# burmajam/delta_crdt_ex

Hardware: AMD Instinct MI355X
Metric: merged dots/sec for AWLWWMap delta join + Merkle diff keys/sec at 1–8 GPUs (higher is better)
Workload: dtype u64; 1 GPU; config2: 1M-key AWLWWMap full-state join of two replicas, 10% concurrent-write conflicts, per GPU (key-hash range shards); keys_per_gpu=1000000, rows_in_per_gpu=2000000, rows_out_per_gpu=1100011, parallelism=key-hash shards x1, rotate=4

## Files before the change

### delta_crdt_ex_amd/csrc/join.hip

```cpp
#include <algorithm>
#include <mutex>

#include "dg_ctxu.h"
#include "dg_launch.h"

namespace dg {

namespace {

constexpr int JB = JOIN_BLOCK;
constexpr int JI = JOIN_ITEMS;
constexpr int JT = JOIN_TILE;
static_assert(JT % 2 == 0, "even tiles (balance_tiles keeps them even)");
constexpr int JS = JT + 5;
constexpr int VT = 64;

#ifdef DG_STAMPS
__device__ u64 g_join_stamps[65536 * 16];
#define JSTAMP(tile, k)                                                              \
  do {                                                                               \
    __syncthreads();                                                                 \
    __builtin_amdgcn_sched_barrier(0);                                               \
    if (threadIdx.x == 0 && (tile) < 65536) g_join_stamps[(tile) * 16 + (k)] =       \
        __builtin_amdgcn_s_memrealtime();                                            \
    __builtin_amdgcn_sched_barrier(0);                                               \
  } while (0)
#else
#define JSTAMP(tile, k) \
  do {                  \
  } while (0)
#endif

constexpr int CB = 1024;

__global__ __launch_bounds__(CB) void ctx_union_kernel(CtxUnionArgs p) {
  __shared__ u32 s_wave[CB / WAVE + 1];
  ctx_union_block<CB>(p, s_wave);
}

struct ChgLayout {
  u64* ev;
  u64* off;
  u32* cnt;
  u32* wu;
  u64* fk;
  u64* lk;
};

static __host__ ChgLayout chg_layout(void* tmp, u64 ntiles) {
  ChgLayout l;
  char* c = (char*)tmp;
  l.ev = (u64*)c;
  c += ntiles * (u64)JT * 8;
  l.off = (u64*)c;
  c += ntiles * 8;
  l.cnt = (u32*)c;
  c += ntiles * 4;
  l.wu = (u32*)c;
  c += ntiles * 4;
  c += ntiles * 4;
  c = (char*)(((uintptr_t)c + 7) & ~(uintptr_t)7);
  l.fk = (u64*)c;
  c += ntiles * 8;
  l.lk = (u64*)c;
  return l;
}

struct JoinArgs {
  Rows a, b;
  Ctx ca, cb;
  const u64* keys;
  u64 n_keys;
  const u64* splits;
  u64* ksplits;
  u64 ntiles;
  u64 jt;
  RowsOut out;
  Scan scan;
  u64* d_count;
  unsigned short* lists;
  u32* counts;
  u64* chg_tmp;
  u32* chg_cnt;
  u32* chg_wu;
  u64* chg_fk;
  u64* chg_lk;
  int fused;
  CtxUnionArgs cu;
};

__device__ __forceinline__ bool mp_pred(const Rows A, const Rows B, u64 diag, u64 i) {
  u64 j = diag - 1 - i;
  u64 ka = A.key[i], kb = B.key[j];
  if (ka != kb) return ka < kb;
  return row_le(load_row(A, i), load_row(B, j));
}

constexpr int PB = 256;
constexpr int PK = 2 * WAVE;

__device__ u64 mp_search(const Rows A, const Rows B, u64 d, u64 lo, u64 hi) {
  const int lane = threadIdx.x & (WAVE - 1);
  for (int round = 0; round < 64 && hi > lo; round++) {
    const u64 span = hi - lo;
    bool f0, f1;
    if (span <= (u64)PK) {
      const u64 x0 = lo + 2 * lane, x1 = x0 + 1;
      f0 = x0 < hi && !mp_pred(A, B, d, x0);
      f1 = x1 < hi && !mp_pred(A, B, d, x1);
    } else {
      const u64 x0 = lo + (span * (u64)(2 * lane + 1)) / (PK + 1);
      const u64 x1 = lo + (span * (u64)(2 * lane + 2)) / (PK + 1);
      f0 = !mp_pred(A, B, d, x0);
      f1 = !mp_pred(A, B, d, x1);
    }
    const u64 m0 = __ballot(f0), m1 = __ballot(f1);
    int kf = PK;
    if (m0 | m1) {
      const int l0 = m0 ? __ffsll((long long)m0) - 1 : 64;
      const int l1 = m1 ? __ffsll((long long)m1) - 1 : 64;
      kf = (l0 <= l1) ? 2 * l0 : 2 * l1 + 1;
    }
    if (span <= (u64)PK) {
      return (u64)kf < span ? lo + kf : hi;
    } else if (kf == PK) {
      lo = lo + (span * (u64)PK) / (PK + 1) + 1;
    } else {
      const u64 nh = lo + (span * (u64)(kf + 1)) / (PK + 1);
      if (kf > 0) lo = lo + (span * (u64)kf) / (PK + 1) + 1;
      hi = nh;
    }
  }
  return lo;
}

__device__ u64 mp_split(const Rows A, const Rows B, u64 d) {
  const int lane = threadIdx.x & (WAVE - 1);
  const u64 na = A.n, nb = B.n, total = na + nb;
  const u64 lo = d > nb ? d - nb : 0, hi = min(d, na);
  if (hi - lo <= (u64)PK) return mp_search(A, B, d, lo, hi);
  const double scale = (double)na * (double)nb / ((double)total * 18446744073709551616.0);
  u64 i = (u64)((double)d * (double)na / (double)total);
  i = min(max(i, lo), hi - 1);
  {
    const double gap = (double)B.key[d - 1 - i] - (double)A.key[i];
    const double lim = (double)(hi - lo);
    double sft = gap * scale;
    sft = sft > lim ? lim : (sft < -lim ? -lim : sft);
    i64 ni = (i64)i + (i64)sft;
    ni = ni < (i64)lo ? (i64)lo : (ni > (i64)hi - 1 ? (i64)hi - 1 : ni);
    i = (u64)ni;
  }
  for (int r = 0; r < 3; r++) {
    constexpr u64 PW = WAVE;
    u64 wlo = i > lo + PW / 2 ? i - PW / 2 : lo;
    const u64 whi = min(wlo + PW, hi);
    wlo = whi - PW > lo ? whi - PW : lo;
    const u64 x0 = wlo + lane;
    const u64 m0 = __ballot(x0 < whi && !mp_pred(A, B, d, x0));
    const u64 kf = m0 ? (u64)(__ffsll((long long)m0) - 1) : whi - wlo;
    if ((kf > 0 || wlo == lo) && (kf < whi - wlo || whi == hi)) return wlo + kf;
    const u64 c = (wlo + whi) / 2;
    const double gap = (double)B.key[d - 1 - c] - (double)A.key[c];
    double sft = gap * scale;
    const double lim = (double)(hi - lo);
    sft = sft > lim ? lim : (sft < -lim ? -lim : sft);
    i64 ni = (i64)c + (i64)sft;
    ni = ni < (i64)lo ? (i64)lo : (ni > (i64)hi - 1 ? (i64)hi - 1 : ni);
    i = (u64)ni;
  }
  return mp_search(A, B, d, lo, hi);
}

__device__ __forceinline__ u64 split_guess(u64 na, u64 nb, u64 d) {
  const u64 lo = d > nb ? d - nb : 0, hi = min(d, na);
  const u64 i = (u64)((double)d * (double)na / (double)(na + nb));
  return min(max(i, lo), hi);
}

__device__ __forceinline__ bool guess_exact(const Rows& A, const Rows& B, u64 d, u64 g) {
  const u64 lo = d > B.n ? d - B.n : 0, hi = min(d, A.n);
  bool ok = true;
  if (g > lo) ok = row_le(load_row(A, g - 1), load_row(B, d - g));
  if (g < hi) ok = ok && !row_le(load_row(A, g), load_row(B, d - 1 - g));
  return ok;
}

__device__ __forceinline__ u64 key_split(const Rows& A, const Rows& B, const u64* keys, u64 n_keys,
                                         u64 d, u64 s) {
  const u64 ib = d - s;
  const bool va = s < A.n, vb = ib < B.n;
  if (!va && !vb) return n_keys;
  const u64 ka = va ? A.key[s] : ~0ull, kb = vb ? B.key[ib] : ~0ull;
  return wave_lower_bound(keys, n_keys, min(ka, kb));
}

__global__ __launch_bounds__(PB) void join2_partition_kernel(Rows A, Rows B, u64 ntiles, u64 jt,
                                                             u64* splits, CtxUnionArgs cu,
                                                             const u64* keys, u64 n_keys,
                                                             u64* ksplits) {
  if (blockIdx.x == 0) {
    __shared__ u32 s_wave[PB / WAVE + 1];
    ctx_union_block<PB>(cu, s_wave);
    return;
  }
  const u64 q = (u64)(blockIdx.x - 1) * (PB / WAVE) + (threadIdx.x >> 6);
  if (q > ntiles) return;
  const u64 d = min(q * jt, A.n + B.n);
  const u64 s = mp_split(A, B, d);
  if ((threadIdx.x & (WAVE - 1)) == 0) splits[q] = s;
  if (keys) {
    const u64 kq = key_split(A, B, keys, n_keys, d, s);
    if ((threadIdx.x & (WAVE - 1)) == 0) ksplits[q] = kq;
  }
}

template <bool FAST>
__device__ __forceinline__ bool covers(const u64* tab, const Ctx& c, u32 dn, u64 dc) {
  if (FAST) {
    if (dn < (u32)VT) return tab[dn] >= dc;
    return ctx_covers(c.node, c.cnt, c.n, 0, dn, dc);
  }
  return ctx_covers(c.node, c.cnt, c.n, c.kind, dn, dc);
}

constexpr int KS = 64;
struct KeySlice {
  const u64* lds;
  const u64* keys;
  u64 km;
};

__device__ __forceinline__ bool key_in(const KeySlice& ks, u64 x) {
  if (ks.lds) {
    const int km = (int)ks.km;
    int pos = 0;
#pragma unroll
    for (int step = KS; step >= 1; step >>= 1) {
      const int m = pos + step;
      const bool c = (m <= km) & (ks.lds[min(m, KS) - 1] < x);
      pos = c ? m : pos;
    }
    return (pos < km) & (ks.lds[min(pos, KS - 1)] == x);
  }
  return keyset_has(ks.keys, ks.km, x);
}

__device__ __forceinline__ bool fill_vv_tables(const Ctx& ca, const Ctx& cb, u64* tab_a, u64* tab_b) {
  bool far = false;
  for (u64 i = threadIdx.x; i < ca.n; i += JB) {
    const u32 nd = ca.node[i];
    if (nd < (u32)VT) tab_a[nd] = ca.cnt[i];
    far |= nd >= (u32)VT;
  }
  for (u64 i = threadIdx.x; i < cb.n; i += JB) {
    const u32 nd = cb.node[i];
    if (nd < (u32)VT) tab_b[nd] = cb.cnt[i];
    far |= nd >= (u32)VT;
  }
  return far;
}

struct Buf {
  alignas(16) u64 kv[JS][2];
  alignas(16) u64 tc[JS][2];
  u32 node[JS];
};

__device__ __forceinline__ u64 buf_key(const Buf& s, int x) { return s.kv[x][0]; }

__device__ __forceinline__ void buf_put(Buf& s, int x, u64 key, u64 val, i64 ts, u32 node, u64 cnt) {
  typedef u64 v2u64 __attribute__((ext_vector_type(2)));
  *(v2u64*)s.kv[x] = v2u64{key, val};
  *(v2u64*)s.tc[x] = v2u64{(u64)ts, cnt};
  s.node[x] = node;
}

__device__ __forceinline__ i64 slot_row(int x, int nat, u64 a0, u64 b0, u64 na, u64 nb,
                                        bool* from_b) {
  if (x < nat + 2) {
    const i64 g = (i64)a0 - 1 + x;
    *from_b = false;
    return (g >= 0 && (u64)g < na) ? g : -1;
  }
  const i64 g = (i64)b0 - 1 + (x - (nat + 2));
  *from_b = true;
  return (g >= 0 && (u64)g < nb) ? g : -1;
}

constexpr int SLOTS = (JS + JB - 1) / JB;

__device__ __forceinline__ Row lds_row(const Buf& s, int x) {
  typedef u64 v2u64 __attribute__((ext_vector_type(2)));
  const v2u64 kv = *(const v2u64*)s.kv[x];
  const v2u64 tc = *(const v2u64*)s.tc[x];
  Row r;
  r.key = kv.x;
  r.val = kv.y;
  r.ts = (i64)tc.x;
  r.cnt = tc.y;
  r.node = s.node[x];
  return r;
}

constexpr int search_top(int n) { return n <= 1 ? 1 : 2 * search_top(n / 2); }
constexpr int STOP = search_top(JT);

template <bool FAST, bool KEYED, bool CHG = false, bool NOFB = false>
__device__ __forceinline__ void merge_items(const Ctx& ca, const Ctx& cb, const u64* tab_a,
                                            const u64* tab_b, const KeySlice& ks,
                                            const u64 nb, const Buf& s, int nat, int nbt, u64 a0,
                                            u64 b0, u32& keep, unsigned short (&src)[JI],
                                            u32* ev = nullptr) {
  const int tid = threadIdx.x;
  const int offB = nat + 2;
  const int tt = nat + nbt;
  const int diag = min(tid * JI, tt);
  const int dend = min(diag + JI, tt);
  const int lo0 = diag > nbt ? diag - nbt : 0, hi0 = min(diag, nat);
  int lo = lo0;
#pragma unroll
  for (int step = STOP; step >= 1; step >>= 1) {
    const int m = lo + step;
    const int mc = min(m, hi0);
    const bool c = (m <= hi0) & (buf_key(s, mc) <= buf_key(s, offB + 1 + diag - mc));
    lo = c ? m : lo;
  }
  int i = lo;
  while (i > lo0 && buf_key(s, i) == buf_key(s, offB + 1 + diag - i)) {
    bool lt, eq;
    row_cmp_bf(lds_row(s, i), lds_row(s, offB + 1 + diag - i), lt, eq);
    if (lt | eq) break;
    i--;
  }
  int j = diag - i;
  Row ra = lds_row(s, 1 + i), rb = lds_row(s, offB + 1 + j);
  bool dup = false;
  if (((a0 + (u64)i) >= 1) && buf_key(s, i) == rb.key) dup = row_eq(lds_row(s, i), rb);
  Row xa = lds_row(s, 2 + i), xb = lds_row(s, offB + 2 + j);
  keep = 0;
  if (CHG) *ev = 0;
#pragma unroll
  for (int k = 0; k < JI; k++) {
    const bool valid = diag + k < dend;
    const bool bvalid = (b0 + (u64)j) < nb;
    bool lt, eq;
    row_cmp_bf(ra, rb, lt, eq);
    const bool takeA = (i < nat) & ((j >= nbt) | lt | eq);
    const bool inB = bvalid & eq;
    bool kp;
    const bool jn = KEYED ? key_in(ks, takeA ? ra.key : rb.key) : true;
    if (FAST) {
      const u32 dn = takeA ? ra.node : rb.node;
      const u64 dc = takeA ? ra.cnt : rb.cnt;
      bool cov;
      if (dn < (u32)VT) {
        cov = (takeA ? tab_b : tab_a)[dn] >= dc;
      } else if (NOFB) {
        cov = dc == 0;
      } else {
        const u32* vn = takeA ? opaque_ptr(cb.node) : opaque_ptr(ca.node);
        const u64* vc = takeA ? opaque_ptr(cb.cnt) : opaque_ptr(ca.cnt);
        const u64 vnn = takeA ? opaque_val(cb.n) : opaque_val(ca.n);
        cov = ctx_covers(vn, vc, vnn, 0, dn, dc);
      }
      if (KEYED) {
        const bool bprev = ((b0 + (u64)j) >= 1) & (buf_key(s, offB + j) == ra.key);
        const bool bnext = bvalid & (rb.key == ra.key);
        kp = takeA ? (jn ? (inB | !cov) : !(bprev | bnext)) : (!jn | (!dup & !cov));
      } else {
        kp = takeA ? (inB || !cov) : (!dup && !cov);
      }
    } else if (takeA) {
      if (jn) {
        kp = inB || !covers<FAST>(tab_b, cb, ra.node, ra.cnt);
      } else {
        const bool bprev = (b0 + (u64)j) >= 1 && buf_key(s, offB + j) == ra.key;
        const bool bnext = bvalid && rb.key == ra.key;
        kp = !(bprev || bnext);
      }
    } else {
      if (jn)
        kp = !dup && !covers<FAST>(tab_a, ca, rb.node, rb.cnt);
      else
        kp = true;
    }
    src[k] = valid ? (unsigned short)(takeA ? 1 + i : offB + 1 + j) : (unsigned short)0;
    if (valid && kp) keep |= 1u << k;
    if (CHG && valid && jn && (takeA ? !kp : kp)) *ev |= 1u << k;
    dup = takeA ? inB : false;
    i += takeA ? 1 : 0;
    j += takeA ? 0 : 1;
    ra = row_sel(takeA, xa, ra);
    rb = row_sel(takeA, rb, xb);
    if (k + 1 < JI) {
      const Row nx = lds_row(s, takeA ? 2 + i : offB + 2 + j);
      xa = row_sel(takeA, nx, xa);
      xb = row_sel(takeA, xb, nx);
    }
  }
}

struct TileLds {
  Buf buf;
  union {
    u64 tab[2][VT];
    unsigned short comp[JT];
  } u;
  u32 wave[JB / WAVE + 1];
  u64 lb[3 * (JB / WAVE) + 2];
  u64 bcast[4];
};

struct Staged {
  u64 k[SLOTS], v[SLOTS], c[SLOTS];
  i64 t[SLOTS];
  u32 n[SLOTS];
  bool ok[SLOTS];
};

__device__ __forceinline__ void tile_geom(u64 t, u64 jt, u64 a0, u64 a1, u64 total, int* nat,
                                          int* nbt, u64* b0) {
  const u64 d0 = t * jt, d1 = min(d0 + jt, total);
  *nat = (int)(a1 - a0);
  *nbt = (int)((d1 - a1) - (d0 - a0));
  *b0 = d0 - a0;
}

__device__ __forceinline__ void issue_tile(const Rows& A, const Rows& B, int nat, int nbt, u64 a0,
                                           u64 b0, Staged& r) {
  const int tid = threadIdx.x;
#pragma unroll
  for (int k = 0; k < SLOTS; k++) {
    const int x = tid + k * JB;
    bool fb = false;
    const i64 g = x < nat + nbt + 4 ? slot_row(x, nat, a0, b0, A.n, B.n, &fb) : -1;
    r.ok[k] = g >= 0;
    if (r.ok[k]) {
      const Row x = load_row_sel(A, B, fb, (u64)g);
      r.k[k] = x.key;
      r.v[k] = x.val;
      r.t[k] = x.ts;
      r.n[k] = x.node;
      r.c[k] = x.cnt;
    }
  }
}

__device__ __forceinline__ void commit_tile(const Staged& r, Buf& s) {
  const int tid = threadIdx.x;
#pragma unroll
  for (int k = 0; k < SLOTS; k++) {
    const int x = tid + k * JB;
    if (r.ok[k]) buf_put(s, x, r.k[k], r.v[k], r.t[k], r.n[k], r.c[k]);
  }
}

constexpr int FUSE_IT = 4;

template <bool KEYED>
struct StreamLds {
  Buf buf[2];
  unsigned short comp[2][JT];
  u64 tab[2][VT];
  u64 kslice[2][KEYED ? KS : 1];
  u64 kspl[KEYED ? 2 * FUSE_IT : 1];
  u32 wave[JB / WAVE + 1];
  u64 red[2][2 * (JB / WAVE)];
  u64 spl[2 * FUSE_IT];
  u64 chk[JB / WAVE];
  int chf[JB / WAVE];
};

constexpr u32 CNT_BITS = 12;
static_assert(JT < (1 << CNT_BITS), "tile count must fit the granule's count field");
constexpr int CQ = (1024 + JB - 1) / JB;
static_assert((u64)CQ * JB + 1 <= JOIN_MAX_GRID, "start flags cover every join grid");

__device__ __forceinline__ void publish_count(u32* cs, u64 t, u32 epoch, u32 n) {
  __hip_atomic_store(cs + t, (epoch << CNT_BITS) | n, __ATOMIC_RELAXED, __HIP_MEMORY_SCOPE_AGENT);
}

struct StripeCounts {
  u32 v[CQ];
  bool ready;
};

__device__ __forceinline__ void stripe_load(const u32* cs, u64 base_t, u64 G, u64 ntiles, u32 epoch,
                                            StripeCounts& c) {
  c.ready = true;
#pragma unroll
  for (int q = 0; q < CQ; q++) {
    const u64 x = (u64)threadIdx.x + (u64)q * JB;
    c.v[q] = epoch << CNT_BITS;
    if (x < G && base_t + x < ntiles)
      c.v[q] = __hip_atomic_load(cs + base_t + x, __ATOMIC_RELAXED, __HIP_MEMORY_SCOPE_AGENT);
  }
}

constexpr u32 ABORT_POLLS = 1u << 13;

template <class T>
__device__ __forceinline__ T cold(const T* field) {
  return *(const volatile T*)field;
}

__device__ __forceinline__ const Scan* cold_scan() {
  return &((const JoinArgs*)__builtin_amdgcn_kernarg_segment_ptr())->scan;
}

__device__ __forceinline__ bool grid_check(u32 epoch, u32 spins, u64 need, const StripeCounts& c) {
  const Scan* sc = cold_scan();
  u32* abort = cold(&sc->abort);
  if (__hip_atomic_load(abort, __ATOMIC_RELAXED, __HIP_MEMORY_SCOPE_AGENT) == epoch) return true;
  if (spins <= ABORT_POLLS) return false;
  const u32* started = cold(&sc->started);
  bool absent = false;
#pragma unroll
  for (int q = 0; q < CQ; q++) {
    const u64 x = (u64)threadIdx.x + (u64)q * JB;
    if (x < need && (c.v[q] >> CNT_BITS) != epoch &&
        __hip_atomic_load(started + x, __ATOMIC_RELAXED, __HIP_MEMORY_SCOPE_AGENT) != epoch)
      absent = true;
  }
  if (!absent) return false;
  __hip_atomic_store(abort, epoch, __ATOMIC_RELAXED, __HIP_MEMORY_SCOPE_AGENT);
  atomicOr(cold(&sc->err), 2u);
  return true;
}

__device__ __forceinline__ void stripe_sums(const u32* cs, u32 epoch, u32* err, u64 base_t,
                                            u64 G, u64 w, bool need_all, StripeCounts& c,
                                            u64* s_red, u64* below, u64* all) {
  const int tid = threadIdx.x;
  const u64 need = need_all ? G : w;
  for (u32 spins = 0;; spins++) {
    bool ready = true;
#pragma unroll
    for (int q = 0; q < CQ; q++)
      ready &= (u64)tid + (u64)q * JB >= need || (c.v[q] >> CNT_BITS) == epoch;
    if (ready) break;
    if ((spins & 63) == 63 && grid_check(epoch, spins, need, c)) {
#pragma unroll
      for (int q = 0; q < CQ; q++)
        if ((c.v[q] >> CNT_BITS) != epoch) c.v[q] = epoch << CNT_BITS;
      break;
    }
    if (spins > (1u << 24)) {
      atomicOr(err, 1u);
      break;
    }
    __builtin_amdgcn_s_sleep(2);
#pragma unroll
    for (int q = 0; q < CQ; q++) {
      const u64 x = (u64)tid + (u64)q * JB;
      if (x < need && (c.v[q] >> CNT_BITS) != epoch)
        c.v[q] = __hip_atomic_load(cs + base_t + x, __ATOMIC_RELAXED, __HIP_MEMORY_SCOPE_AGENT);
    }
  }
  u64 lo = 0, tot = 0;
#pragma unroll
  for (int q = 0; q < CQ; q++) {
    const u64 x = (u64)tid + (u64)q * JB;
    const u64 n = c.v[q] & ((1u << CNT_BITS) - 1);
    tot += n;
    lo += x < w ? n : 0;
  }
  lo = wave_sum_u32((u32)lo);
  tot = wave_sum_u32((u32)tot);
  constexpr int NW = JB / WAVE;
  if ((tid & (WAVE - 1)) == 0) {
    s_red[tid / WAVE] = lo;
    s_red[NW + tid / WAVE] = tot;
  }
  __syncthreads();
  lo = 0;
  tot = 0;
#pragma unroll
  for (int i = 0; i < NW; i++) {
    lo += s_red[i];
    tot += s_red[NW + i];
  }
  *below = lo;
  *all = tot;
}

template <bool KEYED>
__device__ __forceinline__ void write_tile(const JoinArgs& p, const StreamLds<KEYED>& s, int bi,
                                           u64 o0, u32 n) {
  const Buf& b = s.buf[bi];
  for (u32 q = threadIdx.x; q < n; q += JB) {
    const Row x = lds_row(b, s.comp[bi][q]);
    store_row_nt(p.out, o0 + q, x);
  }
}

template <bool FAST, bool KEYED, bool CHG, bool LATE>
__global__ __launch_bounds__(JB) __attribute__((amdgpu_waves_per_eu(4, 8))) void join2_stream_kernel(JoinArgs p) {
  __shared__ StreamLds<KEYED> s;
  const int tid = threadIdx.x;
  const u64 total = p.a.n + p.b.n, ntiles = p.ntiles, w = blockIdx.x;
  const u64 G = gridDim.x - (LATE ? 1 : 0);
  u32* cs = p.scan.counts;
  const u32 epoch = p.scan.epoch;
  const Rows& A = p.a;
  const Rows& B = p.b;
  if (tid == 0)
    __hip_atomic_store(cold(&cold_scan()->started) + w, epoch, __ATOMIC_RELAXED,
                       __HIP_MEMORY_SCOPE_AGENT);
  if (w < G) JSTAMP(w, 0);
  Staged r;
  u64 ga0 = 0, ga1 = 0;
  if (LATE) {
    if (w == G) {
      ctx_union_block<JB>(p.cu, s.wave);
      return;
    }
    {
      ga0 = split_guess(A.n, B.n, w * p.jt);
      ga1 = split_guess(A.n, B.n, min((w + 1) * p.jt, total));
      int gnat, gnbt;
      u64 gb0;
      tile_geom(w, p.jt, ga0, ga1, total, &gnat, &gnbt, &gb0);
      issue_tile(A, B, gnat, gnbt, ga0, gb0, r);
    }
    for (int q = tid / WAVE; q < 2 * FUSE_IT; q += JB / WAVE) {
      const u64 tk = w + (u64)(q >> 1) * G;
      if (tk >= ntiles) break;
      const u64 d = min((tk + (q & 1)) * p.jt, total);
      const u64 g = split_guess(A.n, B.n, d);
      const u64 sp = guess_exact(A, B, d, g) ? g : mp_split(A, B, d);
      if ((tid & (WAVE - 1)) == 0) s.spl[q] = sp;
      if (KEYED) {
        const u64 kq = key_split(A, B, p.keys, p.n_keys, d, sp);
        if ((tid & (WAVE - 1)) == 0) s.kspl[q] = kq;
      }
    }
  }
  if (FAST)
    for (int x = tid; x < 2 * VT; x += JB) (&s.tab[0][0])[x] = 0;
  if (LATE) __syncthreads();
  if (w < G) JSTAMP(w, 8);
  auto split = [&](u64 tile, int k, int side) -> u64 {
    if (LATE) return s.spl[2 * k + side];
    return p.splits[tile + side];
  };
  auto kslice = [&](u64 tile, int k, u64* kl) -> u64 {
    u64 lo, hi;
    if (LATE) {
      lo = s.kspl[2 * k];
      hi = s.kspl[2 * k + 1];
    } else {
      lo = p.ksplits[tile];
      hi = p.ksplits[tile + 1];
    }
    *kl = lo;
    return min(hi + 1, p.n_keys) - lo;
  };
  u64 t = w;
  u64 a0 = split(t, 0, 0), a1 = split(t, 0, 1);
  int nat, nbt;
  u64 b0;
  tile_geom(t, p.jt, a0, a1, total, &nat, &nbt, &b0);
  if (!LATE || a0 != ga0 || a1 != ga1) issue_tile(A, B, nat, nbt, a0, b0, r);
  u64 kl = 0, km = 0, kk = 0;
  if (KEYED) {
    km = kslice(t, 0, &kl);
    if (km <= (u64)KS && (u64)tid < km) kk = p.keys[kl + tid];
  }
  __syncthreads();
  if (w < G) JSTAMP(w, 9);
  bool vv_far = false;
  if (FAST) {
    vv_far = fill_vv_tables(p.ca, p.cb, s.tab[0], s.tab[1]);
    if (LATE) vv_far = __syncthreads_or(vv_far);
  }
  u64 base = 0;
  u32 np = 0;
  for (int k = 0;; k++) {
    const int bi = k & 1;
    if (k > 0) JSTAMP(t, 0);
    JSTAMP(t, 1);
    commit_tile(r, s.buf[bi]);
    if (KEYED && km <= (u64)KS && (u64)tid < km) s.kslice[bi][tid] = kk;
    __syncthreads();
    JSTAMP(t, 2);
    const u64 tn = t + G;
    u64 a0n = 0, a1n = 0, b0n = 0, kln = 0, kmn = 0;
    int natn = 0, nbtn = 0;
    auto issue_next = [&]() {
      a0n = split(tn, k + 1, 0);
      a1n = split(tn, k + 1, 1);
      tile_geom(tn, p.jt, a0n, a1n, total, &natn, &nbtn, &b0n);
      issue_tile(A, B, natn, nbtn, a0n, b0n, r);
      if (KEYED) {
        kmn = kslice(tn, k + 1, &kln);
        if (kmn <= (u64)KS && (u64)tid < kmn) kk = p.keys[kln + tid];
      }
    };
    if (tn < ntiles) issue_next();
    StripeCounts sc;
    if (k > 0) stripe_load(cs, t - G - w, G, ntiles, epoch, sc);
    JSTAMP(t, 7);
    u32 keep, ev = 0;
    unsigned short src[JI];
    const KeySlice ks{KEYED && km <= (u64)KS ? s.kslice[bi] : nullptr, p.keys + kl, km};
    if (LATE && FAST && !vv_far)
      merge_items<FAST, KEYED, CHG, true>(p.ca, p.cb, s.tab[0], s.tab[1], ks, B.n, s.buf[bi], nat,
                                          nbt, a0, b0, keep, src, &ev);
    else
      merge_items<FAST, KEYED, CHG>(p.ca, p.cb, s.tab[0], s.tab[1], ks, B.n, s.buf[bi], nat, nbt, a0,
                                    b0, keep, src, &ev);
    JSTAMP(t, 3);
    u32 n;
    u32 pos = block_excl_scan1<JB>(__popc(keep), s.wave, &n);
#pragma unroll
    for (int q = 0; q < JI; q++)
      if (keep & (1u << q)) s.comp[bi][pos++] = src[q];
    if (tid == 0) publish_count(cs, t, epoch, n);
    __syncthreads();
    if (CHG) {
      const Buf& cb = s.buf[bi];
      const int ne = __popc(ev);
      u64 fkey = 0, lkey = 0;
      u32 diff = 0;
      bool seen = false;
#pragma unroll
      for (int q = 0; q < JI; q++)
        if (ev & (1u << q)) {
          const u64 k = buf_key(cb, src[q]);
          if (seen && k != lkey) diff++;
          if (!seen) fkey = k;
          lkey = k;
          seen = true;
        }
      const int lane = tid & (WAVE - 1), wv = tid / WAVE;
      const u32 mi = wave_incl_max(ne ? (u32)lane + 1 : 0u);
      const u32 mx = wave_prev(mi);
      const u64 pk = __shfl(lkey, mx > 0 ? (int)mx - 1 : 0, WAVE);
      const u32 ml = (u32)__builtin_amdgcn_readlane((int)mi, WAVE - 1);
      const u64 wk = __shfl(lkey, ml > 0 ? (int)ml - 1 : 0, WAVE);
      if (lane == WAVE - 1) {
        s.chf[wv] = (int)ml;
        s.chk[wv] = wk;
      }
      int pm = (int)mx;
      u64 pkey = pk;
      __syncthreads();
      if (pm == 0)
        for (int w2 = wv - 1; w2 >= 0; w2--)
          if (s.chf[w2] > 0) {
            pm = 1;
            pkey = s.chk[w2];
            break;
          }
      if (ne && pm > 0 && fkey != pkey) diff++;
      u32 tot2;
      const u32 sc2 = block_excl_scan1<JB>((diff << 16) | (u32)ne, s.wave, &tot2);
      const u32 n2 = tot2 & 0xffffu, p0 = sc2 & 0xffffu;
      u64* dst = p.chg_tmp + t * (u64)JT;
      u32 p2 = p0;
#pragma unroll
      for (int q = 0; q < JI; q++)
        if (ev & (1u << q)) dst[p2++] = buf_key(cb, src[q]);
      if (tid == 0) {
        p.chg_cnt[t] = n2;
        p.chg_wu[t] = tot2 >> 16;
      }
      if (ne && p0 == 0) p.chg_fk[t] = fkey;
      if (ne && p2 == n2) p.chg_lk[t] = lkey;
    }
    JSTAMP(t, 4);
    if (k > 0) {
      u64 below, all;
      stripe_sums(cs, epoch, p.scan.err, t - G - w, G, w, true, sc, s.red[k & 1], &below, &all);
      JSTAMP(t, 5);
      write_tile(p, s, bi ^ 1, base + below, np);
      base += all;
    }
    JSTAMP(t, 6);
    np = n;
    if (tn >= ntiles) {
      u64 below, all;
      StripeCounts last;
      stripe_load(cs, t - w, G, ntiles, epoch, last);
      stripe_sums(cs, epoch, p.scan.err, t - w, G, w, false, last, s.red[(k + 1) & 1], &below, &all);
      write_tile(p, s, bi, base + below, np);
      if (tid == 0 && t == ntiles - 1) p.d_count[0] = base + below + np;
      break;
    }
    t = tn;
    a0 = a0n;
    a1 = a1n;
    nat = natn;
    nbt = nbtn;
    b0 = b0n;
    kl = kln;
    km = kmn;
    __syncthreads();
  }
}

constexpr int CCH = WAVE;
constexpr int CB2 = 256;
constexpr int CWT = CB2 / WAVE;
constexpr int CEV = (JT + WAVE - 1) / WAVE;

struct ChgSum {
  u64 u;
  u64 has;
  u64 fk, lk;
};

__device__ __forceinline__ ChgSum chg_combine(const ChgSum& L, const ChgSum& R) {
  if (!L.has) return ChgSum{L.u + R.u, R.has, R.fk, R.lk};
  if (!R.has) return L;
  return ChgSum{L.u + R.u - (R.fk == L.lk ? 1ull : 0ull), 1ull, L.fk, R.lk};
}

struct ChgArgs {
  const u64* ev;
  const u32* cnt;
  const u32* wu;
  const u64* fk;
  const u64* lk;
  ChgSum* chunk;
  u64 ntiles;
  u64* out;
  u64 cap;
  u64* d_count;
};

__device__ __forceinline__ ChgSum chg_tile(const ChgArgs& p, u64 t) {
  const u32 n = p.cnt[t];
  if (n == 0) return ChgSum{0, 0, 0, 0};
  return ChgSum{(u64)p.wu[t] + 1, 1, p.fk[t], p.lk[t]};
}

__device__ __forceinline__ ChgSum shfl_down_sum(const ChgSum& x, int d) {
  return ChgSum{__shfl_down(x.u, d, WAVE), __shfl_down(x.has, d, WAVE), __shfl_down(x.fk, d, WAVE),
                __shfl_down(x.lk, d, WAVE)};
}

__device__ ChgSum chg_block_reduce(ChgSum x, ChgSum* s_red) {
  const int lane = threadIdx.x & (WAVE - 1), wv = threadIdx.x / WAVE;
#pragma unroll
  for (int d = 1; d < WAVE; d <<= 1) {
    const ChgSum y = shfl_down_sum(x, d);
    if (lane + d < WAVE) x = chg_combine(x, y);
  }
  if (lane == 0) s_red[wv] = x;
  __syncthreads();
  if (threadIdx.x == 0) {
    ChgSum r = s_red[0];
    for (int i = 1; i < CB2 / WAVE; i++) r = chg_combine(r, s_red[i]);
    s_red[CB2 / WAVE] = r;
  }
  __syncthreads();
  const ChgSum r = s_red[CB2 / WAVE];
  __syncthreads();
  return r;
}

__device__ __forceinline__ ChgSum chg_wave_range(const ChgArgs& p, u64 t0, u64 t1) {
  const int lane = threadIdx.x & (WAVE - 1);
  const u64 t = t0 + lane;
  ChgSum x = t < t1 ? chg_tile(p, t) : ChgSum{0, 0, 0, 0};
#pragma unroll
  for (int d = 1; d < WAVE; d <<= 1) {
    const ChgSum y = shfl_down_sum(x, d);
    if (lane + d < WAVE) x = chg_combine(x, y);
  }
  return ChgSum{__shfl(x.u, 0, WAVE), __shfl(x.has, 0, WAVE), __shfl(x.fk, 0, WAVE),
                __shfl(x.lk, 0, WAVE)};
}

__global__ __launch_bounds__(CB2) void chg_sum_kernel(ChgArgs p, u64 nchunk) {
  const u64 c = (u64)blockIdx.x * (CB2 / WAVE) + threadIdx.x / WAVE;
  if (c >= nchunk) return;
  const ChgSum r = chg_wave_range(p, c * CCH, min(c * CCH + CCH, p.ntiles));
  if ((threadIdx.x & (WAVE - 1)) == 0) p.chunk[c] = r;
}

__global__ __launch_bounds__(CB2) void chg_write_kernel(ChgArgs p) {
  __shared__ ChgSum s_red[CB2 / WAVE + 1];
  __shared__ ChgSum s_tile[CWT];
  __shared__ u64 s_off[CWT];
  __shared__ u32 s_dup[CWT];
  const int tid = threadIdx.x, lane = tid & (WAVE - 1), wv = tid / WAVE;
  const u64 t0 = (u64)blockIdx.x * CWT, chunk = t0 / CCH;
  ChgSum acc{0, 0, 0, 0};
  for (u64 c0 = 0; c0 < chunk; c0 += CB2) {
    const ChgSum x = c0 + tid < chunk ? p.chunk[c0 + tid] : ChgSum{0, 0, 0, 0};
    acc = chg_combine(acc, chg_block_reduce(x, s_red));
  }
  if (wv == 0) {
    const ChgSum in = chg_wave_range(p, chunk * CCH, t0);
    if (lane == 0) s_red[0] = chg_combine(acc, in);
  }
  if (tid < CWT) s_tile[tid] = t0 + tid < p.ntiles ? chg_tile(p, t0 + tid) : ChgSum{0, 0, 0, 0};
  __syncthreads();
  if (tid == 0) {
    ChgSum run = s_red[0];
    for (int i = 0; i < CWT; i++) {
      const ChgSum x = s_tile[i];
      const bool dup = x.has && run.has && x.fk == run.lk;
      s_dup[i] = dup ? 1u : 0u;
      s_off[i] = run.u;
      run = chg_combine(run, x);
    }
    if (t0 + CWT >= p.ntiles) p.d_count[0] = run.u;
  }
  __syncthreads();
  {
    const int i = wv;
    const u64 t = t0 + i;
    if (t >= p.ntiles) return;
    const u32 n = p.cnt[t];
    const u64* ev = p.ev + t * (u64)JT;
    u64 o = s_off[i];
    const bool dup0 = s_dup[i] != 0;
    for (u32 e0 = 0; e0 < n; e0 += WAVE) {
      const u32 e = e0 + lane;
      const u64 k = e < n ? ev[e] : 0;
      const bool keep = e < n && (e > 0 ? ev[e - 1] != k : !dup0);
      const u64 m = __ballot(keep);
      const u64 pos = o + __popcll(m & ((1ull << lane) - 1));
      if (keep && pos < p.cap) p.out[pos] = k;
      o += __popcll(m);
    }
  }
}

template <bool FAST, bool KEYED>
__global__ __launch_bounds__(JB) void join2_slot_kernel(JoinArgs p) {
  __shared__ TileLds s;
  const int tid = threadIdx.x;
  const u64 total = p.a.n + p.b.n;
  if (FAST)
    for (int x = tid; x < 2 * VT; x += JB) (&s.u.tab[0][0])[x] = 0;
  const u64 t = blockIdx.x;
  const u64 a0 = p.splits[t], a1 = p.splits[t + 1];
  int nat, nbt;
  u64 b0;
  tile_geom(t, p.jt, a0, a1, total, &nat, &nbt, &b0);
  Staged r;
  issue_tile(p.a, p.b, nat, nbt, a0, b0, r);
  __syncthreads();
  if (FAST) fill_vv_tables(p.ca, p.cb, s.u.tab[0], s.u.tab[1]);
  JSTAMP(t, 0);
  JSTAMP(t, 1);
  commit_tile(r, s.buf);
  __syncthreads();
  JSTAMP(t, 2);
  u32 keep;
  unsigned short src[JI];
  const KeySlice ks{nullptr, p.keys, p.n_keys};
  merge_items<FAST, KEYED>(p.ca, p.cb, s.u.tab[0], s.u.tab[1], ks, p.b.n, s.buf, nat, nbt, a0, b0,
                           keep, src);
  JSTAMP(t, 3);
  u32 n;
  u32 pos = block_excl_scan<JB>(__popc(keep), s.wave, &n);
#pragma unroll
  for (int q = 0; q < JI; q++)
    if (keep & (1u << q)) s.u.comp[pos++] = src[q];
  __syncthreads();
  JSTAMP(t, 4);
  JSTAMP(t, 5);
  if (tid == 0) p.counts[t] = n;
  for (u32 q = tid; q < n; q += JB) p.lists[t * JT + q] = s.u.comp[q];
  JSTAMP(t, 6);
}

constexpr int CPB = 256;
constexpr int CPU_ = 8;

__global__ __launch_bounds__(CPB) void join2_compact_kernel(Rows a, Rows b, const u64* splits,
                                                            const unsigned short* lists,
                                                            const u32* counts, u64 ntiles,
                                                            RowsOut out, u64* d_count) {
  __shared__ u32 s_wave[CPB / WAVE + 1];
  __shared__ u64 s_pre;
  const u64 tile = blockIdx.x;
  u64 part = 0;
  for (u64 base = 0; base < tile; base += (u64)CPB * CPU_) {
    u32 v[CPU_];
#pragma unroll
    for (int k = 0; k < CPU_; k++) {
      const u64 i = base + (u64)k * CPB + threadIdx.x;
      v[k] = i < tile ? counts[i] : 0u;
    }
#pragma unroll
    for (int k = 0; k < CPU_; k++) part += v[k];
  }
#pragma unroll
  for (int d = WAVE / 2; d >= 1; d >>= 1) part += __shfl_xor(part, d, WAVE);
  if ((threadIdx.x & (WAVE - 1)) == 0) s_wave[threadIdx.x / WAVE] = (u32)part;
  __syncthreads();
  if (threadIdx.x == 0) {
    u64 acc = 0;
    for (int w = 0; w < CPB / WAVE; w++) acc += s_wave[w];
    s_pre = acc;
    if (tile == ntiles - 1) d_count[0] = acc + counts[tile];
  }
  __syncthreads();
  const u64 base = s_pre, n = counts[tile];
  const u64 a0 = splits[tile], a1 = splits[tile + 1];
  const u64 d0 = tile * JT;
  const int nat = (int)(a1 - a0);
  const u64 b0 = d0 - a0;
  for (u64 q = threadIdx.x; q < n; q += CPB) {
    const int x = lists[tile * JT + q];
    const bool fb = x >= nat + 2;
    const u64 g = fb ? b0 - 1 + (u64)(x - nat - 2) : a0 - 1 + (u64)x;
    const Row r = load_row_sel(a, b, fb, g);
    store_row_nt(out, base + q, r);
  }
}

}

static u64 resident_grid(const void* k) {
  struct Entry {
    const void* k;
    int dev;
    u64 n;
  };
  static Entry cache[32];
  static int used = 0;
  static std::mutex mu;
  int dev = 0;
  if (hipGetDevice(&dev) != hipSuccess) return 256;
  {
    std::lock_guard<std::mutex> g(mu);
    for (int i = 0; i < used; i++)
      if (cache[i].k == k && cache[i].dev == dev) return cache[i].n;
  }
  int per_cu = 0, cus = 0;
  if (hipDeviceGetAttribute(&cus, hipDeviceAttributeMultiprocessorCount, dev) != hipSuccess ||
      hipOccupancyMaxActiveBlocksPerMultiprocessor(&per_cu, k, JB, 0) != hipSuccess || per_cu <= 0 ||
      cus <= 0)
    return 256;
  const u64 n = (u64)per_cu * (u64)cus;
  std::lock_guard<std::mutex> g(mu);
  if (used < 32) cache[used++] = {k, dev, n};
  return n;
}

static hipError_t launch_stream(void (*kern)(JoinArgs), u64 grid, JoinArgs& p, hipStream_t st) {
  static const bool coop = [] {
    const char* v = getenv("DG_JOIN_COOP");
    return v && v[0] == '1';
  }();
  if (!coop) {
    hipLaunchKernelGGL(kern, dim3((unsigned)grid), dim3(JB), 0, st, p);
    return hipGetLastError();
  }
  void* args[] = {&p};
  return hipLaunchCooperativeKernel((const void*)kern, dim3((unsigned)grid), dim3(JB), args, 0, st);
}


static void balance_tiles(JoinArgs& p, u64 G) {
  const u64 total = p.a.n + p.b.n;
  if (G == 0 || p.ntiles <= G) return;
  const u64 k = (p.ntiles + G - 1) / G;
  const u64 jt = std::min<u64>(((total + k * G - 1) / (k * G) + 1) & ~1ull, JT);
  p.jt = jt;
  p.ntiles = (total + jt - 1) / jt;
}

hipError_t launch_join2(const Rows& a, const Ctx& ca, const Rows& b, const Ctx& cb,
                        const u64* keys, u64 n_keys, const RowsOut& out, u32* out_ctx_node,
                        u64* out_ctx_cnt, void* ctx_tmp, void* pass_tmp, int mode,
                        const Scan& scan, int workers, u64* d_counts, hipStream_t st,
                        void* chg_tmp) {
  JoinArgs p;
  p.a = a;
  p.b = b;
  p.ca = ca;
  p.cb = cb;
  p.keys = keys;
  p.n_keys = n_keys;
  p.ntiles = join2_tiles(a.n, b.n);
  p.jt = JT;
  auto place_splits = [&]() {
    p.splits = scan.state + p.ntiles;
    p.ksplits = scan.state + 2 * p.ntiles + 1;
  };
  place_splits();
  const CtxUnionArgs cu = make_cu(ca, cb, out_ctx_node, out_ctx_cnt, d_counts + 1, ctx_tmp);
  p.out = out;
  p.scan = scan;
  p.d_count = d_counts;
  p.lists = nullptr;
  p.counts = nullptr;
  p.chg_tmp = chg_tmp ? (u64*)chg_tmp : nullptr;
  p.chg_cnt = p.chg_wu = nullptr;
  p.chg_fk = p.chg_lk = nullptr;
  if (chg_tmp) {
    const ChgLayout l = chg_layout(chg_tmp, p.ntiles);
    p.chg_cnt = l.cnt;
    p.chg_wu = l.wu;
    p.chg_fk = l.fk;
    p.chg_lk = l.lk;
  }
  if (p.ntiles == 0) {
    hipError_t e = hipMemsetAsync(d_counts, 0, sizeof(u64), st);
    if (e != hipSuccess) return e;
    hipLaunchKernelGGL(ctx_union_kernel, dim3(1), dim3(CB), 0, st, cu);
    return hipGetLastError();
  }
  const bool fast = ca.kind == 0 && cb.kind == 0;
  const bool keyed = keys != nullptr;
  p.fused = 0;
  p.cu = cu;
  void (*const kerns[2][2][2][2])(JoinArgs) = {
      {{{join2_stream_kernel<false, false, false, false>, join2_stream_kernel<false, false, false, true>},
        {join2_stream_kernel<false, false, true, false>, join2_stream_kernel<false, false, true, true>}},
       {{join2_stream_kernel<false, true, false, false>, join2_stream_kernel<false, true, false, true>},
        {join2_stream_kernel<false, true, true, false>, join2_stream_kernel<false, true, true, true>}}},
      {{{join2_stream_kernel<true, false, false, false>, join2_stream_kernel<true, false, false, true>},
        {join2_stream_kernel<true, false, true, false>, join2_stream_kernel<true, false, true, true>}},
       {{join2_stream_kernel<true, true, false, false>, join2_stream_kernel<true, true, false, true>},
        {join2_stream_kernel<true, true, true, false>, join2_stream_kernel<true, true, true, true>}}}};
  auto kern = kerns[fast][keyed][chg_tmp != nullptr][0];
  auto kern_late = kerns[fast][keyed][chg_tmp != nullptr][1];
  const bool stream = mode != JOIN_TWO_PASS || chg_tmp;
  u64 g = 0;
  if (stream) {
    g = workers > 0 ? (u64)workers : resident_grid((const void*)kern);
    g = std::min<u64>(std::min<u64>(p.ntiles, g), (u64)CQ * JB);
    static const bool no_fuse = [] {
      const char* v = getenv("DG_JOIN_FUSE");
      return v && v[0] == '0';
    }();
    const u64 gr = workers > 0 ? g + 1 : resident_grid((const void*)kern_late);
    const u64 gt = std::min<u64>(std::min<u64>(p.ntiles, gr - 1), (u64)CQ * JB);
    if (!no_fuse && gr >= 2 && p.ntiles <= (u64)FUSE_IT * gt) {
      if (!chg_tmp) balance_tiles(p, gt);
      place_splits();
      p.fused = 1;
      return launch_stream(kern_late, gt + 1, p, st);
    }
  }
  const u64 nb_part = (p.ntiles + 1 + (PB / WAVE) - 1) / (PB / WAVE);
  hipLaunchKernelGGL(join2_partition_kernel, dim3((unsigned)nb_part + 1), dim3(PB), 0, st, a, b,
                     p.ntiles, p.jt, scan.state + p.ntiles, cu, keys, n_keys, p.ksplits);
  if (!stream) {
    char* t = (char*)pass_tmp;
    p.counts = (u32*)t;
    t += ((p.ntiles * 4 + 255) / 256) * 256;
    p.lists = (unsigned short*)t;
    auto kern = fast ? (keyed ? join2_slot_kernel<true, true> : join2_slot_kernel<true, false>)
                     : (keyed ? join2_slot_kernel<false, true> : join2_slot_kernel<false, false>);
    hipLaunchKernelGGL(kern, dim3((unsigned)p.ntiles), dim3(JB), 0, st, p);
    hipLaunchKernelGGL(join2_compact_kernel, dim3((unsigned)p.ntiles), dim3(CPB), 0, st, a, b,
                       p.splits, p.lists, p.counts, p.ntiles, out, d_counts);
    return hipGetLastError();
  }
  return launch_stream(kern, g, p, st);
}

hipError_t launch_join2_changes(u64 na, u64 nb, void* chg_tmp, u64* out, u64 cap, u64* d_count,
                                hipStream_t st) {
  const u64 ntiles = join2_tiles(na, nb);
  if (ntiles == 0) return hipMemsetAsync(d_count, 0, sizeof(u64), st);
  const ChgLayout l = chg_layout(chg_tmp, ntiles);
  ChgArgs p;
  p.ev = l.ev;
  p.cnt = l.cnt;
  p.wu = l.wu;
  p.fk = l.fk;
  p.lk = l.lk;
  p.chunk = (ChgSum*)l.off;
  p.ntiles = ntiles;
  p.out = out;
  p.cap = cap;
  p.d_count = d_count;
  const u64 nchunk = (ntiles + CCH - 1) / CCH;
  if (nchunk > 1) {
    const u64 nc = nchunk - 1;
    hipLaunchKernelGGL(chg_sum_kernel, dim3((unsigned)((nc + CB2 / WAVE - 1) / (CB2 / WAVE))),
                       dim3(CB2), 0, st, p, nc);
  }
  hipLaunchKernelGGL(chg_write_kernel, dim3((unsigned)((ntiles + CWT - 1) / CWT)), dim3(CB2), 0,
                     st, p);
  return hipGetLastError();
}

hipError_t launch_ctx_union(const Ctx& a, const Ctx& b, u32* out_node, u64* out_cnt,
                            u64* d_count, void* tmp, hipStream_t st) {
  CtxUnionArgs p = make_cu(a, b, out_node, out_cnt, d_count, tmp);
  hipLaunchKernelGGL(ctx_union_kernel, dim3(1), dim3(CB), 0, st, p);
  return hipGetLastError();
}

#ifdef DG_STAMPS
extern "C" int dg_debug_join_stamps(unsigned long long* host, size_t n) {
  if (n > 65536 * 16) n = 65536 * 16;
  return hipMemcpyFromSymbol(host, HIP_SYMBOL(g_join_stamps), n * 8) == hipSuccess ? 0 : -3;
}
#endif

}
```

Measured before the change: 57.37 billion merged dots/s.

## Make tile loads branchless, prefetch next splits, and defer stripe count loads

Tile staging now clamps row indices so every slot issues an unconditional load, with no per-slot validity flags and no predicated LDS stores. This removes divergence and lets the loads be batched. In the non-keyed, non-late path the split boundaries for the tile after next are loaded one iteration ahead. The stripe count loads are moved after the count publish, or after the change-key emission, so they are more likely to observe ready values. Clamped rows write duplicate or garbage data into padding slots, and the abort store now reads the epoch from kernarg, which adds a small risk of subtle correctness problems.

```diff
diff --git a/delta_crdt_ex_amd/csrc/join.hip b/delta_crdt_ex_amd/csrc/join.hip
--- a/delta_crdt_ex_amd/csrc/join.hip
+++ b/delta_crdt_ex_amd/csrc/join.hip
@@ -276,16 +276,14 @@
   s.node[x] = node;
 }
 
-__device__ __forceinline__ i64 slot_row(int x, int nat, u64 a0, u64 b0, u64 na, u64 nb,
+__device__ __forceinline__ u64 slot_row(int x, int nat, u64 a0, u64 b0, u64 na, u64 nb,
                                         bool* from_b) {
-  if (x < nat + 2) {
-    const i64 g = (i64)a0 - 1 + x;
-    *from_b = false;
-    return (g >= 0 && (u64)g < na) ? g : -1;
-  }
-  const i64 g = (i64)b0 - 1 + (x - (nat + 2));
-  *from_b = true;
-  return (g >= 0 && (u64)g < nb) ? g : -1;
+  const bool in_a = x < nat + 2;
+  const i64 g = in_a ? (i64)a0 - 1 + x : (i64)b0 - 1 + (x - (nat + 2));
+  const bool fb = in_a ? na == 0 : nb != 0;
+  const i64 last = (i64)(fb ? nb : na) - 1;
+  *from_b = fb;
+  return (u64)min(max(g, (i64)0), last);
 }
 
 constexpr int SLOTS = (JS + JB - 1) / JB;
@@ -416,7 +414,6 @@
   u64 k[SLOTS], v[SLOTS], c[SLOTS];
   i64 t[SLOTS];
   u32 n[SLOTS];
-  bool ok[SLOTS];
 };
 
 __device__ __forceinline__ void tile_geom(u64 t, u64 jt, u64 a0, u64 a1, u64 total, int* nat,
@@ -427,33 +424,28 @@
   *b0 = d0 - a0;
 }
 
-__device__ __forceinline__ void issue_tile(const Rows& A, const Rows& B, int nat, int nbt, u64 a0,
-                                           u64 b0, Staged& r) {
+__device__ __forceinline__ void issue_tile(const Rows& A, const Rows& B, int nat, u64 a0, u64 b0,
+                                           Staged& r) {
   const int tid = threadIdx.x;
+  const u64 na = opaque_val(A.n), nb = opaque_val(B.n);
 #pragma unroll
   for (int k = 0; k < SLOTS; k++) {
-    const int x = tid + k * JB;
-    bool fb = false;
-    const i64 g = x < nat + nbt + 4 ? slot_row(x, nat, a0, b0, A.n, B.n, &fb) : -1;
-    r.ok[k] = g >= 0;
-    if (r.ok[k]) {
-      const Row x = load_row_sel(A, B, fb, (u64)g);
-      r.k[k] = x.key;
-      r.v[k] = x.val;
-      r.t[k] = x.ts;
-      r.n[k] = x.node;
-      r.c[k] = x.cnt;
-    }
+    bool fb;
+    const u64 g = slot_row(tid + k * JB, nat, a0, b0, na, nb, &fb);
+    const Row x = load_row_sel(A, B, fb, g);
+    r.k[k] = x.key;
+    r.v[k] = x.val;
+    r.t[k] = x.ts;
+    r.n[k] = x.node;
+    r.c[k] = x.cnt;
   }
 }
 
 __device__ __forceinline__ void commit_tile(const Staged& r, Buf& s) {
   const int tid = threadIdx.x;
 #pragma unroll
-  for (int k = 0; k < SLOTS; k++) {
-    const int x = tid + k * JB;
-    if (r.ok[k]) buf_put(s, x, r.k[k], r.v[k], r.t[k], r.n[k], r.c[k]);
-  }
+  for (int k = 0; k < SLOTS; k++)
+    buf_put(s, min(tid + k * JB, JS - 1), r.k[k], r.v[k], r.t[k], r.n[k], r.c[k]);
 }
 
 constexpr int FUSE_IT = 4;
@@ -492,9 +484,9 @@
 #pragma unroll
   for (int q = 0; q < CQ; q++) {
     const u64 x = (u64)threadIdx.x + (u64)q * JB;
-    c.v[q] = epoch << CNT_BITS;
-    if (x < G && base_t + x < ntiles)
-      c.v[q] = __hip_atomic_load(cs + base_t + x, __ATOMIC_RELAXED, __HIP_MEMORY_SCOPE_AGENT);
+    const bool has = x < G && base_t + x < ntiles;
+    c.v[q] = __hip_atomic_load(cs + base_t + (has ? x : 0), __ATOMIC_RELAXED,
+                               __HIP_MEMORY_SCOPE_AGENT);
   }
 }
 
@@ -524,15 +516,20 @@
       absent = true;
   }
   if (!absent) return false;
-  __hip_atomic_store(abort, epoch, __ATOMIC_RELAXED, __HIP_MEMORY_SCOPE_AGENT);
+  __hip_atomic_store(abort, cold(&sc->epoch), __ATOMIC_RELAXED, __HIP_MEMORY_SCOPE_AGENT);
   atomicOr(cold(&sc->err), 2u);
   return true;
 }
 
 __device__ __forceinline__ void stripe_sums(const u32* cs, u32 epoch, u32* err, u64 base_t,
-                                            u64 G, u64 w, bool need_all, StripeCounts& c,
-                                            u64* s_red, u64* below, u64* all) {
+                                            u64 G, u64 ntiles, u64 w, bool need_all,
+                                            StripeCounts& c, u64* s_red, u64* below, u64* all) {
   const int tid = threadIdx.x;
+#pragma unroll
+  for (int q = 0; q < CQ; q++) {
+    const u64 x = (u64)tid + (u64)q * JB;
+    c.v[q] = x < G && base_t + x < ntiles ? c.v[q] : epoch << CNT_BITS;
+  }
   const u64 need = need_all ? G : w;
   for (u32 spins = 0;; spins++) {
     bool ready = true;
@@ -551,11 +548,12 @@
       break;
     }
     __builtin_amdgcn_s_sleep(2);
+    const u32* cs_poll = cold(&cold_scan()->counts);
 #pragma unroll
     for (int q = 0; q < CQ; q++) {
       const u64 x = (u64)tid + (u64)q * JB;
       if (x < need && (c.v[q] >> CNT_BITS) != epoch)
-        c.v[q] = __hip_atomic_load(cs + base_t + x, __ATOMIC_RELAXED, __HIP_MEMORY_SCOPE_AGENT);
+        c.v[q] = __hip_atomic_load(cs_poll + base_t + x, __ATOMIC_RELAXED, __HIP_MEMORY_SCOPE_AGENT);
     }
   }
   u64 lo = 0, tot = 0;
@@ -622,7 +620,7 @@
       int gnat, gnbt;
       u64 gb0;
       tile_geom(w, p.jt, ga0, ga1, total, &gnat, &gnbt, &gb0);
-      issue_tile(A, B, gnat, gnbt, ga0, gb0, r);
+      issue_tile(A, B, gnat, ga0, gb0, r);
     }
     for (int q = tid / WAVE; q < 2 * FUSE_IT; q += JB / WAVE) {
       const u64 tk = w + (u64)(q >> 1) * G;
@@ -659,10 +657,18 @@
   };
   u64 t = w;
   u64 a0 = split(t, 0, 0), a1 = split(t, 0, 1);
+  constexpr bool AHEAD = !LATE && !KEYED;
+  u64 sa0 = 0, sa1 = 0;
+  auto splits_ahead = [&](u64 tile) {
+    const u64 tq = min(tile, ntiles - 1);
+    sa0 = p.splits[tq];
+    sa1 = p.splits[tq + 1];
+  };
+  if (AHEAD) splits_ahead(t + G);
   int nat, nbt;
   u64 b0;
   tile_geom(t, p.jt, a0, a1, total, &nat, &nbt, &b0);
-  if (!LATE || a0 != ga0 || a1 != ga1) issue_tile(A, B, nat, nbt, a0, b0, r);
+  if (!LATE || a0 != ga0 || a1 != ga1) issue_tile(A, B, nat, a0, b0, r);
   u64 kl = 0, km = 0, kk = 0;
   if (KEYED) {
     km = kslice(t, 0, &kl);
@@ -689,18 +695,20 @@
     u64 a0n = 0, a1n = 0, b0n = 0, kln = 0, kmn = 0;
     int natn = 0, nbtn = 0;
     auto issue_next = [&]() {
-      a0n = split(tn, k + 1, 0);
-      a1n = split(tn, k + 1, 1);
+      a0n = AHEAD ? sa0 : split(tn, k + 1, 0);
+      a1n = AHEAD ? sa1 : split(tn, k + 1, 1);
+      if (AHEAD) asm volatile("" : "+v"(a0n), "+v"(a1n) : : "memory");
       tile_geom(tn, p.jt, a0n, a1n, total, &natn, &nbtn, &b0n);
-      issue_tile(A, B, natn, nbtn, a0n, b0n, r);
+      issue_tile(A, B, natn, a0n, b0n, r);
+      if (AHEAD) splits_ahead(tn + G);
       if (KEYED) {
         kmn = kslice(tn, k + 1, &kln);
-        if (kmn <= (u64)KS && (u64)tid < kmn) kk = p.keys[kln + tid];
+        const u64 kls = ((u64)__builtin_amdgcn_readfirstlane((int)(kln >> 32)) << 32) |
+                        (u32)__builtin_amdgcn_readfirstlane((int)kln);
+        if (kmn <= (u64)KS && (u64)tid < kmn) kk = (p.keys + kls)[tid];
       }
     };
     if (tn < ntiles) issue_next();
-    StripeCounts sc;
-    if (k > 0) stripe_load(cs, t - G - w, G, ntiles, epoch, sc);
     JSTAMP(t, 7);
     u32 keep, ev = 0;
     unsigned short src[JI];
@@ -718,6 +726,8 @@
     for (int q = 0; q < JI; q++)
       if (keep & (1u << q)) s.comp[bi][pos++] = src[q];
     if (tid == 0) publish_count(cs, t, epoch, n);
+    StripeCounts sc;
+    if (!CHG && k > 0) stripe_load(cs, t - G - w, G, ntiles, epoch, sc);
     __syncthreads();
     if (CHG) {
       const Buf& cb = s.buf[bi];
@@ -769,11 +779,13 @@
       }
       if (ne && p0 == 0) p.chg_fk[t] = fkey;
       if (ne && p2 == n2) p.chg_lk[t] = lkey;
+      if (k > 0) stripe_load(cs, t - G - w, G, ntiles, epoch, sc);
     }
     JSTAMP(t, 4);
     if (k > 0) {
       u64 below, all;
-      stripe_sums(cs, epoch, p.scan.err, t - G - w, G, w, true, sc, s.red[k & 1], &below, &all);
+      stripe_sums(cs, epoch, p.scan.err, t - G - w, G, ntiles, w, true, sc, s.red[k & 1], &below,
+                  &all);
       JSTAMP(t, 5);
       write_tile(p, s, bi ^ 1, base + below, np);
       base += all;
@@ -784,7 +796,8 @@
       u64 below, all;
       StripeCounts last;
       stripe_load(cs, t - w, G, ntiles, epoch, last);
-      stripe_sums(cs, epoch, p.scan.err, t - w, G, w, false, last, s.red[(k + 1) & 1], &below, &all);
+      stripe_sums(cs, epoch, p.scan.err, t - w, G, ntiles, w, false, last, s.red[(k + 1) & 1],
+                  &below, &all);
       write_tile(p, s, bi, base + below, np);
       if (tid == 0 && t == ntiles - 1) p.d_count[0] = base + below + np;
       break;
@@ -945,7 +958,7 @@
   u64 b0;
   tile_geom(t, p.jt, a0, a1, total, &nat, &nbt, &b0);
   Staged r;
-  issue_tile(p.a, p.b, nat, nbt, a0, b0, r);
+  issue_tile(p.a, p.b, nat, a0, b0, r);
   __syncthreads();
   if (FAST) fill_vv_tables(p.ca, p.cb, s.u.tab[0], s.u.tab[1]);
   JSTAMP(t, 0);
```

New measurement: 60.09 billion merged dots/s, median of 6. 1.05x the previous value.
